# gooofy/zerovox

Measured on AMD Instinct MI355X. Metric: audio samples/sec + RTF, 128-phoneme zero-shot synth @22.05kHz, 1/2/4/8 GPU, higher is better.
Workload: dtype f16+bf16

## Files before the change

### zerovox_amd/csrc/gemm.hip

```cpp
#include "mfma_util.h"
#include "zvx_kernels.h"

#include <cstring>
#include <type_traits>

#ifndef ZVX_GEMM_PART
#define ZVX_GEMM_PART 0
#endif
#define ZVX_PART_MAIN (ZVX_GEMM_PART != 2)
#define ZVX_PART_RESFUSE (ZVX_GEMM_PART != 1)
#if ZVX_GEMM_PART == 2
extern thread_local bool zvx_gemm_dry_run;
#else
thread_local hipEvent_t zvx_gemm_ev_start = nullptr, zvx_gemm_ev_stop = nullptr;
thread_local bool zvx_gemm_dry_run = false;
#endif
#define g_dry_run zvx_gemm_dry_run

#define ZVX_LAUNCH(...) do { if (!g_dry_run) ZVX_DISPATCH(__VA_ARGS__); } while (0)

namespace zvx {


#define PITCH 80
// ... 478 lines not shown
    }
#pragma unroll
    for (int j = 0; j < TM; j++)
#pragma unroll
        for (int p = 0; p < NP; p++) {
            const int r = row_base + j * 32 + p * RPP + lane / LPR;
            if (r < a.M && r < out_len && nok) *(u32x4*)(obase + (long)r * a.ldo) = o[j][p];
        }
}

#if ZVX_PART_MAIN
#define SLAB_KC 64
#define SLAB_PITCH 144

__global__ void k_pack_w(const unsigned short* w, int ntaps, int N, int K, unsigned short* out, int nkc, long total_frag_lanes) {
    long idx = (long)blockIdx.x * blockDim.x + threadIdx.x;
    if (idx >= total_frag_lanes) return;
    const int lane = idx & 63; long t = idx >> 6;
    const int k16 = t & 3; t >>= 2;
    const int tap = t % ntaps; t /= ntaps;
    const int kc = t % nkc; const int nt = t / nkc;
    const int n = nt * 32 + (lane & 31);
    const int k0 = kc * SLAB_KC + k16 * 16 + 8 * (lane >> 5);
    unsigned short v[8];
#pragma unroll
    for (int e = 0; e < 8; e++) {
        const int k = k0 + e;
        v[e] = (n < N && k < K) ? w[((long)tap * N + n) * K + k] : (unsigned short)0;
    }
    uint4 o;
    o.x = v[0] | ((unsigned)v[1] << 16); o.y = v[2] | ((unsigned)v[3] << 16);
    o.z = v[4] | ((unsigned)v[5] << 16); o.w = v[6] | ((unsigned)v[7] << 16);
    *(uint4*)(out + idx * 8) = o;
}

size_t packed_weight_elems(int ntaps, int N, int K) {
    const int nkc = (K + SLAB_KC - 1) / SLAB_KC, nt = (N + 31) / 32;
    return (size_t)nt * nkc * ntaps * 4 * 64 * 8;
}
void launch_pack_weights(const void* w_bf16, int ntaps, int N, int K, void* out, hipStream_t s) {
    const int nkc = (K + SLAB_KC - 1) / SLAB_KC, nt = (N + 31) / 32;
    const long total = (long)nt * nkc * ntaps * 4 * 64;
    hipLaunchKernelGGL(k_pack_w, dim3((unsigned)((total + 255) / 256)), dim3(256), 0, s, (const unsigned short*)w_bf16, ntaps, N, K,
                       (unsigned short*)out, nkc, total);
}

void launch_pack_pair(const void* packedA, int ntapsA, int KA, const void* packedB, int ntapsB, int KB, int N, void* out, hipStream_t s) {
    const size_t nt = (N + 31) / 32;
    const size_t szA = (size_t)((KA + SLAB_KC - 1) / SLAB_KC) * ntapsA * 4 * 1024, szB = (size_t)((KB + SLAB_KC - 1) / SLAB_KC) * ntapsB * 4 * 1024;
    (void)hipMemcpy2DAsync(out, szA + szB, packedA, szA, szA, nt, hipMemcpyDeviceToDevice, s);
    (void)hipMemcpy2DAsync((char*)out + szA, szA + szB, packedB, szB, szB, nt, hipMemcpyDeviceToDevice, s);
}

template <int BM, int BN, int WM, int WN, bool FULLK, int MINW, int R, int EPI = -1, int MAXH = 64, bool F16 = false>
__global__ __launch_bounds__(256, MINW) void convslab_kernel(const GemmArgs a) {
    constexpr int TM = BM / WM / 32, TN = BN / WN / 32;
    constexpr int NIT = ((BM + MAXH) * 8 + 255) / 256;
    static_assert(WM * WN == 4, "4 waves");
    extern __shared__ __attribute__((aligned(16))) unsigned char slab[];
    if (F16 && EPI >= 0 && EPI != ZVX_EPI(0, 0, 1) && EPI != ZVX_EPI_FLIP) f16_saturate_mode();

    const int tid = threadIdx.x, lane = tid & 63, wave = __builtin_amdgcn_readfirstlane(tid >> 6);
    const int wr = wave % WM, wc = wave / WM;
    const int ntn = (a.N + BN - 1) / BN;
    int wg, b;
    if (a.xcd_flat) {
        const int nx = gridDim.x, nwg = nx * gridDim.y, id = blockIdx.y * nx + blockIdx.x, q = nwg >> 3, r = nwg & 7, xcd = id & 7;
        const int w = (xcd < r ? xcd * (q + 1) : r * (q + 1) + (xcd - r) * q) + (id >> 3);
        b = w / nx; wg = w - b * nx;
    } else {
        const int nwg = gridDim.x, id = blockIdx.x, q = nwg >> 3, r = nwg & 7, xcd = id & 7;
        wg = (xcd < r ? xcd * (q + 1) : r * (q + 1) + (xcd - r) * q) + (id >> 3);
        b = blockIdx.y;
    }
    const int nt = wg % ntn, mt = wg / ntn;
    const int m0 = mt * BM, n0 = nt * BN;
    const bool bflat = a.bflat != 0;
    const int out_len = bflat ? a.M : (a.out_len ? a.out_len[b] : a.M);
    const int in_len = bflat ? 0 : (a.in_len ? a.in_len[b] : a.in_len_static);
    if (m0 >= out_len || m0 >= a.M) return;
    if (bflat) {
        const int b0 = m0 / a.bflat, t0 = m0 - b0 * a.bflat;
        if (t0 >= a.out_len[b0] && t0 + BM <= a.bflat) return;
    }

    const int HL = a.halo_l, SR = BM + a.halo_l + a.halo_r;
    const int nkc = (a.K + SLAB_KC - 1) / SLAB_KC, n16 = a.K >> 4, ntaps = a.ntaps;
    const unsigned short* Xp = (const unsigned short*)a.X + (long)b * a.x_bs;
    const int nkc2 = (!FULLK && a.K2 > 0) ? (a.K2 + SLAB_KC - 1) / SLAB_KC : 0, n16_2 = a.K2 >> 4;
    const unsigned short* Xp2 = (const unsigned short*)a.X2 + (long)b * a.x2_bs;
    const int in_rows = ((MAXH > 64 || bflat) && a.flat_win) ? a.flat_rows : in_len;
    unsigned rowmask = 0xffffffffu;
    if (bflat) {
        rowmask = 0;
#pragma unroll
        for (int it = 0; it < NIT; it++) {
            const int g = m0 - HL + ((tid + it * 256) >> 3);
            if (g >= 0 && g < in_rows) { const int bb = g / a.bflat; if (g - bb * a.bflat < a.in_len[bb]) rowmask |= 1u << it; }
        }
    } else if (MAXH > 64 && a.flat_win) {
        rowmask = 0;
#pragma unroll
        for (int it = 0; it < NIT; it++) {
            const int g = m0 - HL + ((tid + it * 256) >> 3);
            if (g >= 0 && g < in_rows && (g % a.flat_win) < in_len) rowmask |= 1u << it;
        }
    }
// ... 2 lines not shown
#pragma unroll
    for (int i = 0; i < TN; i++)
#pragma unroll
        for (int j = 0; j < TM; j++)
#pragma unroll
            for (int e = 0; e < 16; e++) acc[i][j][e] = 0.f;

    constexpr bool WREG = R == 0;
    constexpr int F = BN / 32, CNT = F >= 4 ? F / 4 : 1, WD = 4, D = WREG ? WD : R - 1, WAITN = WREG ? (WD - 1) * TN : (D - 2) * CNT;
    const int nt32_total = (a.N + 31) >> 5;
    const int nsteps = a.ntaps * 4, gtotal = nkc * nsteps + nkc2 * 4;
    const uint4* wsrc[CNT];
#pragma unroll
    for (int j = 0; j < CNT; j++) {
        const int f = wave * CNT + j, t32 = (n0 >> 5) + f;
        wsrc[j] = (const uint4*)a.Wp + (long)(t32 < nt32_total ? t32 : 0) * gtotal * 64 + lane;
    }
    const int xrow0 = HL + wr * (BM / WM) + (lane & 31);
    const int koff = (lane >> 5) * 16;
    unsigned char* ring = slab + ((SR * SLAB_PITCH + 1023) & ~1023);
    const unsigned lds_base = (unsigned)(size_t)(__attribute__((address_space(3))) unsigned char*)slab;
    const int dvreg = a.dv[lane & (ZVX_MAX_TAPS - 1)];
    const bool loader = wave * CNT < F;
    const unsigned char* wq[TN];
#pragma unroll
    for (int i = 0; i < TN; i++) {
        const int t32 = (n0 >> 5) + wc * TN + i;
        wq[i] = (const unsigned char*)a.Wp + (long)(t32 < nt32_total ? t32 : 0) * gtotal * 1024;
    }
    const bool wave_dead = __builtin_amdgcn_readfirstlane((int)(n0 + wc * TN * 32 >= a.N)) != 0;
    const unsigned lane16 = lane * 16;
    u32x4 wreg[WREG ? WD : 1][TN] = {};
    auto wload = [&](int gs, int slot) {
        const long off = (long)(gs < gtotal ? gs : gtotal - 1) * 1024;
#pragma unroll
        for (int i = 0; i < TN; i++)
            asm volatile("global_load_dwordx4 %0, %1, %2" : "+v"(wreg[WREG ? slot : 0][i]) : "v"(lane16), "s"(wq[i] + off) : "memory");
    };
    auto dma = [&](int gs) {
        if (WREG || !loader) return;
        const int slot = gs & (R - 1);
        const long off = (long)(gs < gtotal ? gs : gtotal - 1) * 64;
#pragma unroll
        for (int j = 0; j < CNT; j++)
            __builtin_amdgcn_global_load_lds((const __attribute__((address_space(1))) void*)(wsrc[j] + off),
                                             (__attribute__((address_space(3))) void*)(ring + (slot * F + wave * CNT + j) * 1024), 16, 0, 0);
    };
    if (WREG) { wload(0, 0); wload(1, 1); wload(2, 2); wload(3, 3); }
    else {
#pragma unroll
        for (int s0 = 0; s0 < D; s0++) dma(s0);
    }

    for (int kc = 0; kc < nkc + nkc2; kc++) {
        const bool src2 = !FULLK && kc >= nkc;
        const unsigned short* const Xs = src2 ? Xp2 : Xp;
        const int ldxs = src2 ? a.ldx2 : a.ldx, Ks = src2 ? a.K2 : a.K, kbase = (src2 ? kc - nkc : kc) * SLAB_KC;
        {
            constexpr int FCH = NIT > 10 ? (NIT + 1) / 2 : NIT;
#pragma unroll
            for (int h0 = 0; h0 < NIT; h0 += FCH) {
                uint4 sv[FCH];
#pragma unroll
                for (int i = 0; i < FCH; i++) {
                    const int it = h0 + i;
                    const int c = tid + it * 256;
                    const int row = c >> 3, q = c & 7;
                    const int g = m0 - HL + row, k = kbase + q * 8;
                    sv[i] = make_uint4(0, 0, 0, 0);
                    if (it < NIT && c < SR * 8 && g >= 0 && g < in_rows && k < Ks && ((rowmask >> it) & 1)) sv[i] = *(const uint4*)(Xs + (long)g * ldxs + k);
                }
                if (kc && h0 == 0) __syncthreads();
#pragma unroll
                for (int i = 0; i < FCH; i++) {
                    const int c = tid + (h0 + i) * 256;
                    if (h0 + i < NIT && c < SR * 8) *(uint4*)(slab + (c >> 3) * SLAB_PITCH + (c & 7) * 16) = sv[i];
                }
            }
        }
        __syncthreads();
        int nk16 = 4;
        if (!FULLK) { nk16 = src2 ? n16_2 - (kc - nkc) * 4 : n16 - kc * 4; if (nk16 > 4) nk16 = 4; if (wave_dead) nk16 = 0; }
        const int ntaps_kc = src2 ? 1 : ntaps;

        uint4 xA[TM], wA[TN], xB[TM], wB[TN];
        const unsigned ring_rd = lds_base + (unsigned)(size_t)(ring - slab) + lane * 16 + wc * TN * 1024;
        const int gs0 = src2 ? nkc * nsteps + (kc - nkc) * 4 : kc * nsteps;
        auto rd = [&](uint4 (&xf)[TM], uint4 (&wf)[TN], int gs, unsigned rowoff, int kk) {
            if (!WREG) {
                const unsigned wa = ring_rd + (gs & ((WREG ? 1 : R) - 1)) * (F * 1024);
#pragma unroll
                for (int i = 0; i < TN; i++)
                    asm volatile("ds_read_b128 %0, %1 offset:%2" : "=v"(wf[i]) : "v"(wa), "n"(i * 1024));
            }
#pragma unroll
            for (int j = 0; j < TM; j++)
                asm volatile("ds_read_b128 %0, %1" : "=v"(xf[j]) : "v"(lds_base + rowoff + j * 32 * SLAB_PITCH + kk * 32));
        };
        auto mma = [&](uint4 (&xf)[TM], uint4 (&wf)[TN]) {
#pragma unroll
            for (int i = 0; i < TN; i++)
#pragma unroll
                for (int j = 0; j < TM; j++)
                    acc[i][j] = F16 ? __builtin_amdgcn_mfma_f32_32x32x16_f16(__builtin_bit_cast(f16x8, wf[i]), __builtin_bit_cast(f16x8, xf[j]), acc[i][j], 0, 0, 0)
                                    : __builtin_amdgcn_mfma_f32_32x32x16_bf16(__builtin_bit_cast(bf16x8, wf[i]),
                                                                       __builtin_bit_cast(bf16x8, xf[j]), acc[i][j], 0, 0, 0);
        };
        auto mma_r = [&](uint4 (&xf)[TM], int slot) {
#pragma unroll
            for (int i = 0; i < TN; i++)
#pragma unroll
                for (int j = 0; j < TM; j++)
                    acc[i][j] = F16 ? __builtin_amdgcn_mfma_f32_32x32x16_f16(__builtin_bit_cast(f16x8, wreg[WREG ? slot : 0][i]), __builtin_bit_cast(f16x8, xf[j]), acc[i][j], 0, 0, 0)
                                    : __builtin_amdgcn_mfma_f32_32x32x16_bf16(__builtin_bit_cast(bf16x8, wreg[WREG ? slot : 0][i]),
                                                                       __builtin_bit_cast(bf16x8, xf[j]), acc[i][j], 0, 0, 0);
        };
        auto rowoff_of = [&](int tap) {
            const int d = src2 ? 0 : __builtin_amdgcn_readlane(dvreg, tap < ntaps ? tap : ntaps - 1);
            return (unsigned)((xrow0 + d) * SLAB_PITCH + koff);
        };
        unsigned rowoff = rowoff_of(0);
        rd(xA, wA, gs0, rowoff, 0);
        for (int tap = 0; tap < ntaps_kc; tap++) {
            const unsigned rowoff_next = rowoff_of(tap + 1);
#pragma unroll
            for (int kk = 0; kk < 4; kk++) {
                const int gs = gs0 + tap * 4 + kk;
                if (WREG) asm volatile("s_waitcnt vmcnt(%0)" :: "n"(WAITN) : "memory");
                else asm volatile("s_waitcnt vmcnt(%0)\n\ts_barrier" :: "n"(WAITN) : "memory");
                dma(gs + D);
                if (kk & 1) rd(xA, wA, gs + 1, kk == 3 ? rowoff_next : rowoff, (kk + 1) & 3);
                else        rd(xB, wB, gs + 1, rowoff, kk + 1);
                asm volatile("s_waitcnt lgkmcnt(%0)" :: "n"(WREG ? TM : TM + TN) : "memory");
                __builtin_amdgcn_sched_barrier(0);
                if (FULLK || kk < nk16) {
                    if (WREG) { if (kk & 1) mma_r(xB, kk); else mma_r(xA, kk); }
                    else { if (kk & 1) mma(xB, wB); else mma(xA, wA); }
                }
                __builtin_amdgcn_sched_barrier(0);
                if (WREG) wload(gs + WD, kk);
            }
            rowoff = rowoff_next;
        }
        asm volatile("s_waitcnt lgkmcnt(0)" ::: "memory");
    }
    if (WREG) {
#pragma unroll
        for (int sl = 0; sl < (WREG ? WD : 1); sl++)
#pragma unroll
            for (int i = 0; i < TN; i++) asm volatile("s_waitcnt vmcnt(0)" : "+v"(wreg[sl][i]) :: "memory");
    } else {
        asm volatile("s_waitcnt vmcnt(0)" ::: "memory");
    }
    __syncthreads();
    if (EPI == ZVX_EPI_FLIP)
        epilogue_direct<TM, TN, !F16>(a, acc, b, m0 + wr * (BM / WM), n0 + wc * (BN / WN), out_len, lane, slab + wave * (32 * (TN * 64 + 16)));
    else if (EPI == ZVX_EPI(0, 0, 1))
        epilogue_direct<TM, TN, F16>(a, acc, b, m0 + wr * (BM / WM), n0 + wc * (BN / WN), out_len, lane, slab + wave * (32 * (TN * 64 + 16)));
    else
        epilogue_rows<TM, TN, 0, EPI, (F16 && EPI >= 0)>(a, acc, b, m0 + wr * (BM / WM), n0 + wc * (BN / WN), out_len, lane, slab + wave * (32 * (TN * 32 * 4 + 16)));
}

template <int C, int NT, int BM, int WM, int WN, int MINW, int MAXH = 64, bool F16 = false>
__global__ __launch_bounds__(256, MINW) void convreg_kernel(const GemmArgs a) {
    constexpr int TM = BM / WM / 32;
    constexpr int KS = C / 16;
    constexpr int PITCH_ = C * 2 + 16;
    constexpr int CPR = C / 8;
    constexpr int NIT = ((BM + MAXH) * CPR + 255) / 256;
    constexpr int FCH = NIT > 12 ? 8 : NIT;
    static_assert(WM * WN == 4 && WN * 32 == C, "wave layout");
    extern __shared__ __attribute__((aligned(16))) unsigned char slab[];

    const int tid = threadIdx.x, lane = tid & 63, wave = tid >> 6;
    const int wr = wave % WM, wc = wave / WM;
    int wg;
    {
        const int nwg = gridDim.x, id = blockIdx.x, q = nwg >> 3, r = nwg & 7, xcd = id & 7;
        wg = (xcd < r ? xcd * (q + 1) : r * (q + 1) + (xcd - r) * q) + (id >> 3);
    }
    const int m0 = wg * BM, b = blockIdx.y;
    const int out_len = a.out_len ? a.out_len[b] : a.M;
    const int in_len = a.in_len ? a.in_len[b] : a.in_len_static;
    if (m0 >= out_len || m0 >= a.M) return;
    const int HL = a.halo_l, SR = BM + a.halo_l + a.halo_r;
    const unsigned short* Xp = (const unsigned short*)a.X + (long)b * a.x_bs;

    uint4 w[NT][KS];
    {
        const uint4* Wq = (const uint4*)a.Wp + ((long)wc * NT * 4) * 64 + lane;
#pragma unroll
        for (int t = 0; t < NT; t++)
#pragma unroll
            for (int kk = 0; kk < KS; kk++) w[t][kk] = Wq[(t * 4 + kk) * 64];
    }
    {
        const bool flat = MAXH > 64 && a.flat_win;
// ... 882 lines not shown
    a.fused = 1;
    if (a.N == 128 && a.no_pairstream != 1) {
        const int h2 = (a.ntaps - 1) / 2, dil = a.dv1[1] - a.dv1[0];
        bool ok = a.alpha == 1.f && a.bias_mode == 1 && !a.post_scale && (!a.out || a.out_dtype == a.dtype) && a.res_mode == 2 && a.res_dtype == a.dtype &&
                  a.res == a.X && a.r_bs == a.x_bs && a.ldr == a.ldx && (!a.accum || a.accum_dtype == a.dtype) && (a.act == ACT_NONE || a.act == ACT_LRELU) &&
                  (a.accum_mode || a.out_scale == 1.f) && a.in_len == a.out_len;
        for (int t = 0; t < a.ntaps; t++) ok = ok && a.dv[t] == t - h2 && a.dv1[t] == (t - h2) * dil;
        if (ok) {
            PairArgs p;
            memset(&p, 0, sizeof p);
            p.X = a.X; p.x_bs = a.x_bs; p.ldx = a.ldx; p.W1 = a.Wp2; p.W2 = a.Wp; p.b1 = a.bias1; p.b2 = a.bias;
            p.C = a.N; p.ntaps = a.ntaps; p.dil = dil;
            p.out = a.out; p.o_bs = a.o_bs; p.ldo = a.ldo;
            p.accum = a.accum; p.a_bs = a.a_bs; p.lda = a.lda; p.accum_mode = a.accum ? a.accum_mode : 0;
            p.slope1 = a.slope1; p.res_inv_slope = a.res_inv_slope; p.out_scale = a.out_scale; p.slope = a.act == ACT_LRELU ? a.slope : 1.f;
            p.f16 = a.dtype == DT_F16;
            p.len = a.out_len; p.M = a.M; p.nbatch = a.nbatch; p.force = a.no_pairstream == 2;
            if (launch_pairstream(p, stream, g_dry_run)) return 23;
        }
    }
    {
        if (a.N == 32 && launch_resfuse_persist_c<32>(a, stream)) return 16;
        if (a.N == 64 && a.ntaps != 11 && launch_resfuse_persist_c<64>(a, stream)) return 17;
        if (a.N == 64 && a.ntaps == 11 && launch_resfuse_persist_c<64, 1>(a, stream)) return 17;
    }
    return -1;
}
#endif
#if ZVX_PART_MAIN

struct Variant { const char* name; int dt, bm, bn; };
static const Variant kVariants[] = {
    {"gemm_bf16_128x128", DT_BF16, 128, 128}, {"gemm_bf16_256x64", DT_BF16, 256, 64},
    {"gemm_bf16_256x32", DT_BF16, 256, 32},   {"gemm_f32_128x128", DT_F32, 128, 128},
    {"gemm_f32_256x64", DT_F32, 256, 64},     {"gemm_f32_256x32", DT_F32, 256, 32},
    {"convslab_bf16_128x256", DT_BF16, 128, 256}, {"convslab_bf16_256x128", DT_BF16, 256, 128},
    {"convslab_bf16_256x64", DT_BF16, 256, 64},   {"convslab_bf16_256x32", DT_BF16, 256, 32},
    {"(unused)", DT_BF16, 0, 0}, {"resfuse_bf16_c8", DT_BF16, 256, 8}, {"resfuse_bf16_c16", DT_BF16, 256, 16}, {"resfuse_bf16_c128", DT_BF16, 64, 128},
    {"convreg_bf16_c32", DT_BF16, 512, 32},       {"convreg_bf16_c64", DT_BF16, 256, 64},
    {"resfuse_bf16_c32", DT_BF16, 256, 32},       {"resfuse_bf16_c64", DT_BF16, 128, 64},
    {"gemm_bf16_64x64", DT_BF16, 64, 64},         {"gemm_f32_64x64", DT_F32, 64, 64},
    {"resstream_bf16_c32", DT_BF16, 64, 32},      {"resstream_bf16_c64", DT_BF16, 32, 64},
    {"convslab_bf16_128x128", DT_BF16, 128, 128},
    {"pairstream_bf16_c128", DT_BF16, 128, 128},
    {"narrowstage_c16", DT_BF16, 256, 16}, {"narrowstage_c8", DT_BF16, 512, 8},
    {"conv2d_persist_c32", DT_BF16, 384, 32}, {"conv2d_persist_c64", DT_BF16, 256, 64},
    {"conv2d_s2_c32", DT_BF16, 256, 64}, {"conv2d_s2_c64", DT_BF16, 128, 128},
    {"rb2fuse_bf16_c32", DT_BF16, 256, 32}, {"rb2fuse_bf16_c64", DT_BF16, 256, 64},
};
const char* gemm_variant_name(int id) { return kVariants[id].name; }
int gemm_num_variants() { return (int)(sizeof(kVariants) / sizeof(kVariants[0])); }


template <int BM, int BN, int WM, int WN, int MINW, int R, int EPI = -1>
static void launch_slab_variant(const GemmArgs& a, dim3 grid, size_t lds, hipStream_t stream) {
    const bool fullk = a.K % SLAB_KC == 0 && a.K2 == 0;
    if constexpr (R == 0 || EPI == -1 || EPI == ZVX_EPI(0, 0, 1) || EPI == ZVX_EPI_FLIP) {
        if (a.dtype == DT_F16) {
            if (fullk) ZVX_LAUNCH((convslab_kernel<BM, BN, WM, WN, true, MINW, R, EPI, 64, true>), grid, dim3(256), lds, stream, a);
            else if constexpr (EPI != ZVX_EPI_FLIP) ZVX_LAUNCH((convslab_kernel<BM, BN, WM, WN, false, MINW, R, EPI, 64, true>), grid, dim3(256), lds, stream, a);
            return;
        }
    }
    if constexpr (EPI < 0 || !(EPI & 16)) {
        if (fullk) ZVX_LAUNCH((convslab_kernel<BM, BN, WM, WN, true, MINW, R, EPI>), grid, dim3(256), lds, stream, a);
        else if constexpr (EPI != ZVX_EPI_FLIP) ZVX_LAUNCH((convslab_kernel<BM, BN, WM, WN, false, MINW, R, EPI>), grid, dim3(256), lds, stream, a);
    }
}

int gemm_epi_mode_of(const GemmArgs& a) {
    if (a.alpha == 1.f && !a.post_scale && a.out && a.out_dtype != a.dtype && a.dtype != DT_F32 && a.out_dtype != DT_F32 && !a.out_split3 && a.bias_mode == 1 && a.bias &&
        (a.act == ACT_NONE || a.act == ACT_LRELU) && !a.res_mode && !(a.accum && a.accum_mode) && a.out_scale == 1.f && a.K % SLAB_KC == 0 && !a.K2) return ZVX_EPI_FLIP;
    if (a.alpha != 1.f || a.post_scale || (a.out && a.out_dtype != a.dtype) || a.dtype == DT_F32 || a.out_split3 || a.bias_mode == 2) return -1;
    const int am = a.accum ? a.accum_mode : 0;
    if (a.dtype == DT_F16 && a.out && !am && a.act == ACT_NONE && a.res_mode <= 1 && (!a.res_mode || a.res_dtype == DT_F16) && (a.res_mode || a.out_scale != 1.f) &&
        (a.bias_mode == 0 || a.bias)) return ZVX_EPI_DEC(a.res_mode ? 1 : 0);
    if (a.bias_mode != 1 || !a.bias) return -1;
    if (a.act != ACT_NONE && a.act != ACT_LRELU) return -1;
    if (a.res_mode && (a.res_mode != 2 || a.res_dtype != a.dtype)) return -1;
    if (am && a.accum_dtype != a.dtype) return -1;
    if (!am && a.out_scale != 1.f) return -1;
    if (!a.out && !(am & 2)) return -1;
    const int e = ZVX_EPI(a.res_mode ? 1 : 0, am, a.out ? 1 : 0);
    switch (e) {
        case ZVX_EPI(0, 0, 1): case ZVX_EPI(1, 0, 1): case ZVX_EPI(1, 2, 0): case ZVX_EPI(1, 3, 0): case ZVX_EPI(1, 1, 1): return e;
    }
    return -1;
}

static int launch_convslab(GemmArgs a, hipStream_t stream) {
    const bool bflat_hint = a.bflat != 0;
    if (a.K2) {
        if (!a.X2 || a.K2 % 16 || a.ldx2 % 8 || a.flat_win || (a.bflat && a.x2_bs != (long)a.bflat * a.ldx2)) return -5;
    }
    if (a.bflat) {
        int h = 0;
        for (int i = 0; i < a.ntaps; i++) { const int d = a.dv[i] < 0 ? -a.dv[i] : a.dv[i]; if (d > h) h = d; }
        const bool ok = a.in_len && a.out_len && a.nbatch > 1 && a.bflat >= a.M + h && a.x_bs == (long)a.bflat * a.ldx && (!a.out || a.o_bs == (long)a.bflat * a.ldo) &&
                        (!a.res_mode || a.r_bs == (long)a.bflat * a.ldr) && !a.accum_mode && a.bias_mode != 2 && !a.flat_win && a.M > 128 && a.N >= 128 &&
                        (long)a.nbatch * a.bflat < (1l << 30);
        if (!ok) a.bflat = 0;
    }
    const int g_slab_small = a.slab_small & 7;
    int hl = 0, hr = 0;
    for (int i = 0; i < a.ntaps; i++) { hl = a.dv[i] < -hl ? -a.dv[i] : hl; hr = a.dv[i] > hr ? a.dv[i] : hr; }
    a.halo_l = hl; a.halo_r = hr;
    if (a.flat_win && !a.bflat) {
        if (a.N == a.K && (a.N == 32 || a.N == 64) && !(a.slab_small & 32) && a.dtype == DT_BF16 && a.ntaps == 9 && a.in_len && !a.out_len && hl == a.flat_win + 1 && hr == hl &&
            a.flat_win >= 64 && (long)a.flat_rows * a.ldx * 2 < 0x7fffffffL &&
// ... 229 lines not shown
```

### zerovox_amd/csrc/zvx.hip

```cpp
#include "../../include/zvx.h"
#include "zvx_kernels.h"

#include <dlfcn.h>
#include <math.h>
#include <cmath>
#include <rccl/rccl.h>
#include <stdarg.h>
#include <stdio.h>
#include <string.h>

#include <algorithm>
#include <map>
#include <sstream>
#include <stdexcept>
#include <string>
#include <vector>

using namespace zvx;

namespace {

struct ZvxError : std::runtime_error {
    int code;
    ZvxError(int c, const std::string& m) : std::runtime_error(m), code(c) {}
// ... 36 lines not shown
    hipStream_t front_stream = nullptr;
    hipEvent_t ev_front_done = nullptr, ev_mel_free = nullptr, ev_main_join = nullptr;
    int front_overlap = 1;
    bool mel_free_pending = false;
    bool front_dirty_main = true;
    struct HostSlot { void* p = nullptr; size_t cap = 0; hipEvent_t ready = nullptr, done = nullptr; bool pending = false; int B = 0, pcm16 = 0; long stride = 0, need = 0; };
    HostSlot host_slot[2];
    int host_next = 0, host_last = -1;
    hipStream_t copy_stream = nullptr;
    bool copy_is_comm = false;
    hipStream_t aux_stream = nullptr;
    hipEvent_t ev_aux[2] = {nullptr, nullptr};
    int va_overlap_maxb = 1 << 20;
    ncclComm_t comm = nullptr;
    int rank = 0, world = 1;
    hipEvent_t ev_compute = nullptr;
    std::map<const void*, hipEvent_t> gather_fence;
    std::string err;
    std::map<std::string, std::string> cfg;
    std::map<std::string, Tensor> tensors;
    std::vector<float> host_blob;
    std::map<std::string, DevBuf> bufs;
    std::map<const void*, const void*> packed;
    std::map<const void*, const void*> pair_packed;
    int dt = DT_BF16;
    int H = 0, emb_dim = 0, punct_dim = 0, n_phone_rows = 0, n_punct_rows = 0, max_txt_len = 0, max_mel_len = 0;
    int enc_layers = 0, enc_heads = 0, ffn_dim = 0, ffn_k0 = 0, ffn_k1 = 0, vp_dim = 0, vp_k = 0, n_bins = 0;
    int dec_layers = 0, dec_heads = 0, dec_scln = 0, n_mels = 0, hop = 0, res_dim = 0, dec_kind = 0, rn_asp = 1;
    std::vector<int> rn_layers, rn_filters, voc_rates, voc_ksizes, voc_rb_k;
    std::vector<std::vector<int>> voc_rb_d;
    int voc_resblock = 1, voc_c0 = 0;
    int B = 0, Tmax = 0, Lmax = 0;
    std::vector<int> T_host, mel_len_host;
    std::vector<int> in_stage;
    bool have_features = false, have_mel = false;
    int profile = 0;
    int profile_only = -1;
    int rs_prof = 0;
    int enc_split = 0;
    const void* fft_xs_ready = nullptr;
    int norm_fuse_maxb = 1 << 20;
    int dec_sc_fuse = 1;
    int dec_flat = 1;
    int voc_f16_stages = -1;
    int voc_h16_ok = -1;
    int voc_f16 = 1;
    int dec_f16 = 1;
    int use_attn_f32 = 1;
    int use_flash = 1;
    int use_resstream = 1;
    int rs_seg_min = 0;
    int spk_s2_fuse = 1;
    int spk_pool_fuse = 1;
    int slab_small = 2, slab_flat = 1;
    int poison_pads = 0;
    int sat_check = 0;
    unsigned long long* sat_count_dev() { return (unsigned long long*)buf("sat.count", 64); }
    void sat_scan(const void* x, int dt, long bs, int ld, int B, int rows_max, const int* rows, int C) {
        if (sat_check && x && dt == DT_F16) launch_count_sat16(x, bs, ld, B, rows_max, rows, C, sat_count_dev(), stream);
    }
    int use_rb2fuse = 1;
    int use_stagefuse = 1;
    struct NsWeights { void* W = nullptr; float* bias = nullptr; int woff[18] = {0}; };
    std::map<std::string, NsWeights> ns_weights;
    int use_pairstream = 1;
    int shape_log = 0;
    int max_frames = 1 << 18;
    int out_rate = 0;
    struct RsBank { int L = 0, M = 0, half = 0, T = 0, pitch = 0; const float* dev = nullptr; };
    std::map<std::pair<int, int>, RsBank> rs_banks;
    std::map<int, const double*> lim_wins;
    std::map<int, LoudCoef> loud_coefs;
    void* join_host = nullptr;
    size_t join_host_cap = 0;
    void* join_pinned(size_t bytes) {
        if (bytes > join_host_cap) {
            if (join_host) { HIPCHK(hipStreamSynchronize(stream)); HIPCHK(hipHostFree(join_host)); join_host = nullptr; join_host_cap = 0; }
            const size_t cap = bytes + bytes / 8 + 256;
            HIPCHK(hipHostMalloc(&join_host, cap, hipHostMallocDefault));
            join_host_cap = cap;
        }
        return join_host;
    }
    hipEvent_t stage_ev[ZVX_T_COUNT][2];
    bool stage_used[ZVX_T_COUNT];
    float stage_ms[ZVX_T_COUNT];
    std::vector<GemmEvent> pending;
    std::vector<zvx_kernel_stat> stats;
    std::string tag = "other";
    std::map<std::string, zvx_kernel_stat> tagstats;
    std::map<std::string, zvx_kernel_stat> namedstats;
    std::vector<hipEvent_t> event_pool;

    int cfg_int(const char* k) const {
        auto it = cfg.find(k);
        if (it == cfg.end()) fail(ZVX_E_MANIFEST, "manifest: missing cfg '%s'", k);
        return atoi(it->second.c_str());
    }
    std::vector<int> cfg_list(const char* k) const {
        auto it = cfg.find(k);
        if (it == cfg.end()) fail(ZVX_E_MANIFEST, "manifest: missing cfg '%s'", k);
        std::vector<int> v; std::stringstream ss(it->second); std::string tok;
        while (std::getline(ss, tok, ',')) if (!tok.empty()) v.push_back(atoi(tok.c_str()));
        return v;
    }
    const Tensor& t(const std::string& name) const {
// ... 46 lines not shown
    }
    void arena_end() {
        Arena& a = arena[arena_i];
        if (!a.cur || !stream) return;
        if (!a.ev) HIPCHK(hipEventCreateWithFlags(&a.ev, hipEventDisableTiming));
        HIPCHK(hipEventRecord(a.ev, stream));
        a.pending = true;
        arena_i ^= 1;
    }
    void upload(void* dst, const void* src, size_t bytes) {
        Arena& a = arena[arena_i];
        const size_t need = (bytes + 63) & ~(size_t)63;
        if (!a.p) { HIPCHK(hipHostMalloc((void**)&a.p, ARENA_BYTES, hipHostMallocDefault)); a.cap = ARENA_BYTES; }
        if (a.cur + need > a.cap) {
            HIPCHK(hipMemcpyAsync(dst, src, bytes, hipMemcpyHostToDevice, stream));
            HIPCHK(hipStreamSynchronize(stream));
            return;
        }
        memcpy(a.p + a.cur, src, bytes);
        HIPCHK(hipMemcpyAsync(dst, a.p + a.cur, bytes, hipMemcpyHostToDevice, stream));
        a.cur += need;
    }
    int* upload_ints(const std::string& name, const int* v, size_t n) {
        int* d = ibuf(name, n);
        upload(d, v, n * sizeof(int));
        return d;
    }
    size_t es() const { return dtype_size(dt); }

    hipEvent_t new_event() {
        hipEvent_t e;
        if (!event_pool.empty()) { e = event_pool.back(); event_pool.pop_back(); return e; }
        HIPCHK(hipEventCreate(&e));
        return e;
    }
    void stage_begin(int s) { if (profile) { HIPCHK(hipEventRecord(stage_ev[s][0], stream)); } }
    void stage_end(int s) { if (profile) { HIPCHK(hipEventRecord(stage_ev[s][1], stream)); stage_used[s] = true; } }

    template <typename V, typename L, typename D>
    void profiled(V&& vid, L&& launch, D&& describe) {
        const bool prof = profile >= 2 && (profile_only < 0 || vid() == profile_only);
        if (!prof) { launch(); return; }
        GemmEvent ev{};
        ev.a = new_event(); ev.b = new_event();
        struct Armed { Armed(hipEvent_t a, hipEvent_t b) { profile_events(a, b); } ~Armed() { profile_events(nullptr, nullptr); } };
        ev.variant = [&] { Armed armed(ev.a, ev.b); return launch(); }();
        describe(ev);
        ev.tag = tag;
        pending.push_back(ev);
    }
    void gemm(GemmArgs& a) {
        if (a.flops <= 0) a.flops = 2.0 * (double)a.M * a.nbatch * a.nheads * (double)a.N * ((double)a.K * a.ntaps + (double)a.K2);
        if (!a.Wp && a.dtype != DT_F32) { auto it = packed.find(a.W); if (it != packed.end()) a.Wp = it->second; }
        a.slab_small = slab_small | (spk_s2_fuse ? 0 : 32); a.xcd_flat = slab_flat;
        profiled([&] { return gemm_variant_of(a); }, [&] {
            const int id = a.fused == 2 ? launch_rb2fuse(a, stream) : (a.fused ? launch_resfuse(a, stream) : launch_gemm(a, stream));
            if (id < 0) fail(ZVX_E_INVALID, "launch_gemm rejected shape M=%d N=%d K=%d taps=%d", a.M, a.N, a.K, a.ntaps);
            return id;
        }, [&](GemmEvent& ev) {
            ev.flops = a.flops; ev.rows = (long)a.M * a.nbatch * a.nheads; ev.N = a.N; ev.K = a.K; ev.taps = a.ntaps; ev.res = a.res_mode; ev.fused = a.fused;
            const double esz = dtype_size(a.dtype);
            const double cells = (double)a.M * a.nbatch * a.nheads * a.N;
            ev.bytes = ((double)a.M * a.nbatch * a.nheads) * (double)(a.K + a.K2) * esz + (double)a.N * ((double)a.K * a.ntaps + a.K2) * esz * (a.fused ? 2 : 1) +
                       (a.out ? cells * dtype_size(a.out_dtype) : 0.0) + ((a.res_mode && !a.fused) ? cells * dtype_size(a.res_dtype) : 0.0) +
                       ((a.accum && (a.accum_mode & 1)) ? cells * dtype_size(a.accum_dtype) : 0.0) + ((a.accum && (a.accum_mode & 2)) ? cells * dtype_size(a.accum_dtype) : 0.0);
        });
        if (sat_check && a.nheads == 1) {
            sat_scan(a.out, a.out_dtype, a.o_bs, a.ldo, a.nbatch, a.M, a.out_len, a.N);
            if (a.accum && (a.accum_mode & 2)) sat_scan(a.accum, a.accum_dtype, a.a_bs, a.lda, a.nbatch, a.M, a.out_len, a.N);
        }
    }
    bool run_stream(StreamArgs& a) {
        const int id = launch_resstream(a, this->stream, true);
        if (id < 0) return false;
        profiled([&] { return id; }, [&] {
            const int id2 = launch_resstream(a, this->stream, false);
            if (id2 < 0) fail(ZVX_E_INVALID, "launch_resstream rejected a shape its dry run accepted (C=%d k=%d pairs=%d)", a.C, a.ntaps, a.npair);
            return id2;
        }, [&](GemmEvent& ev) {
            const double rows = (double)a.M * a.nbatch;
            ev.flops = 2.0 * 2.0 * a.npair * rows * a.C * a.C * a.ntaps; ev.rows = (long)rows; ev.N = a.C; ev.K = a.C; ev.taps = a.ntaps;
            ev.res = a.accum_mode; ev.fused = 10 + a.npair;
            ev.bytes = rows * a.C * 2.0 * (1 + (a.out ? 1 : 0) + ((a.accum && (a.accum_mode & 1)) ? 1 : 0) + ((a.accum && (a.accum_mode & 2)) ? 1 : 0));
        });
        return true;
    }
    template <typename F>
    void timed(double flops, double bytes, F&& f, const char* kname = nullptr) {
        const bool prof = profile >= 2 && profile_only < 0;
        GemmEvent ev{};
        if (prof) { ev.a = new_event(); ev.b = new_event(); HIPCHK(hipEventRecord(ev.a, stream)); }
        f();
        if (prof) { HIPCHK(hipEventRecord(ev.b, stream)); ev.variant = -1; ev.flops = flops; ev.bytes = bytes; ev.tag = tag; if (kname) ev.kname = kname; pending.push_back(ev); }
    }
    void resolve_events() {
        if (stats.empty()) {
            stats.resize(gemm_num_variants());
            for (int i = 0; i < gemm_num_variants(); i++) { memset(&stats[i], 0, sizeof stats[i]); snprintf(stats[i].name, 64, "%s", gemm_variant_name(i)); }
        }
        for (auto& e : pending) {
            float ms = 0.f;
            HIPCHK(hipEventElapsedTime(&ms, e.a, e.b));
            if (shape_log && e.variant >= 0) fprintf(stderr, "launch %-24s rows=%-8ld N=%-4d K=%-4d taps=%-2d res=%d fused=%d  %8.3f ms %8.1f TF/s %8.1f GB/s(alg)\n",
                                   gemm_variant_name(e.variant), e.rows, e.N, e.K, e.taps, e.res, e.fused, ms, e.flops / ms / 1e9, e.bytes / ms / 1e6);
            else if (shape_log) fprintf(stderr, "launch %-24s [%s]  %8.3f ms %8.1f GB/s(alg)\n", "(helper)", e.tag.c_str(), ms, e.bytes / ms / 1e6);
            if (e.variant >= 0) { auto& s = stats[e.variant]; s.launches++; s.ms += ms; s.flops += e.flops; s.bytes += e.bytes; }
            auto& ts = tagstats[e.tag];
// ... 2092 lines not shown
    for (auto& hs : c->host_slot) { if (hs.p) (void)hipHostFree(hs.p); if (hs.ready) (void)hipEventDestroy(hs.ready); if (hs.done) (void)hipEventDestroy(hs.done); }
    if (c->join_host) (void)hipHostFree(c->join_host);
    for (int i = 0; i < 2; i++) if (c->voc_aux[i]) { (void)hipStreamSynchronize(c->voc_aux[i]); (void)hipStreamDestroy(c->voc_aux[i]); }
    for (int i = 0; i < 3; i++) if (c->voc_ev[i]) (void)hipEventDestroy(c->voc_ev[i]);
    if (c->aux_stream) { (void)hipStreamSynchronize(c->aux_stream); (void)hipStreamDestroy(c->aux_stream); (void)hipEventDestroy(c->ev_aux[0]); (void)hipEventDestroy(c->ev_aux[1]); }
    if (c->front_stream) {
        (void)hipStreamSynchronize(c->front_stream); (void)hipStreamDestroy(c->front_stream);
        (void)hipEventDestroy(c->ev_front_done); (void)hipEventDestroy(c->ev_mel_free); (void)hipEventDestroy(c->ev_main_join);
    }
    for (auto& kv : c->bufs) if (kv.second.base) (void)hipFree(kv.second.base);
    for (auto e : c->event_pool) (void)hipEventDestroy(e);
    if (c->stream) {
        for (int s = 0; s < ZVX_T_COUNT; s++) { (void)hipEventDestroy(c->stage_ev[s][0]); (void)hipEventDestroy(c->stage_ev[s][1]); }
        (void)hipStreamDestroy(c->stream);
    }
    delete c;
}

const char* zvx_last_error(const zvx_ctx* c) { return c ? c->err.c_str() : g_create_error.c_str(); }

namespace {

struct Switch { const char* key; int zvx_ctx::*v; bool (*ok)(int64_t); };
bool flag(int64_t v) { return v == 0 || v == 1; }
bool count(int64_t v) { return v >= 0 && v <= INT32_MAX; }
const Switch kSwitches[] = {
    {"profile", &zvx_ctx::profile, [](int64_t v) { return v >= 0 && v <= 2; }},
    {"profile_only", &zvx_ctx::profile_only, [](int64_t v) { return v >= -1 && v < gemm_num_variants(); }},
    {"shape_log", &zvx_ctx::shape_log, flag},
    {"rs_prof", &zvx_ctx::rs_prof, flag},
    {"f16_sat_check", &zvx_ctx::sat_check, flag},
    {"poison_pads", &zvx_ctx::poison_pads, flag},
    {"max_frames", &zvx_ctx::max_frames, [](int64_t v) { return v >= 1 && v <= (1 << 24); }},
    {"enc_split", &zvx_ctx::enc_split, [](int64_t v) { return v >= 0 && v <= 2; }},
    {"attn_f32", &zvx_ctx::use_attn_f32, flag},
    {"flash", &zvx_ctx::use_flash, flag},
    {"front_overlap", &zvx_ctx::front_overlap, [](int64_t v) { return v >= 0 && v <= 2; }},
    {"va_overlap_maxb", &zvx_ctx::va_overlap_maxb, count},
    {"dec_f16", &zvx_ctx::dec_f16, flag},
    {"dec_flat", &zvx_ctx::dec_flat, flag},
    {"dec_sc_fuse", &zvx_ctx::dec_sc_fuse, flag},
    {"norm_fuse_maxb", &zvx_ctx::norm_fuse_maxb, count},
    {"voc_f16", &zvx_ctx::voc_f16, flag},
    {"voc_f16_stages", &zvx_ctx::voc_f16_stages, [](int64_t v) { return v >= -1 && v <= INT32_MAX; }},
    {"voc_overlap_maxb", &zvx_ctx::voc_overlap_maxb, count},
    {"voc_overlap_frames", &zvx_ctx::voc_overlap_frames, count},
    {"stagefuse", &zvx_ctx::use_stagefuse, flag},
    {"rb2fuse", &zvx_ctx::use_rb2fuse, flag},
    {"resstream", &zvx_ctx::use_resstream, flag},
    {"rs_seg_min", &zvx_ctx::rs_seg_min, [](int64_t v) { return v >= -1 && v <= INT32_MAX; }},
    {"pairstream", &zvx_ctx::use_pairstream, [](int64_t v) { return v == -1 || v == 0 || v == 1 || v == 3; }},
    {"slab_small", &zvx_ctx::slab_small, [](int64_t v) { return (v & ~32) >= 0 && (v & ~32) <= 2; }},
    {"slab_flat", &zvx_ctx::slab_flat, flag},
    {"spk_pool_fuse", &zvx_ctx::spk_pool_fuse, flag},
    {"spk_s2_fuse", &zvx_ctx::spk_s2_fuse, flag},
    {"out_rate", &zvx_ctx::out_rate, count},
};
const Switch* find_switch(const char* key) {
    for (const Switch& s : kSwitches) if (!strcmp(s.key, key)) return &s;
    return nullptr;
}

}

int64_t zvx_get_int(const zvx_ctx* c, const char* key) {
    if (!c || !key) return -1;
    if (const Switch* s = find_switch(key)) return c->*s->v;
    const std::string k(key);
    if (k == "precision") return c->dt == DT_F32 ? 1 : 0;
    if (k == "hidden") return c->H;
    if (k == "n_mels") return c->n_mels;
    if (k == "hop") return c->hop;
    if (k == "device") return c->device;
    if (k == "dec_kind") return c->dec_kind;
    if (k == "Lmax") return c->Lmax;
    if (k == "f16_sat_events") {
        zvx_ctx* m = const_cast<zvx_ctx*>(c);
        unsigned long long n = 0;
        if (hipSetDevice(m->device) != hipSuccess) return -1;
        try { unsigned long long* d = m->sat_count_dev(); m->sync(); if (hipMemcpy(&n, d, sizeof n, hipMemcpyDeviceToHost) != hipSuccess) return -1; } catch (...) { return -1; }
        return (int64_t)n;
    }
    if (k == "host_slot") return c->host_last;
    if (k.rfind("variant_id:", 0) == 0) { for (int i = 0; i < gemm_num_variants(); i++) if (k.substr(11) == gemm_variant_name(i)) return i; return -1; }
    auto it = c->cfg.find(k);
    if (it != c->cfg.end()) return atoll(it->second.c_str());
    return -1;
}

zvx_status zvx_set_int(zvx_ctx* c, const char* key, int64_t value) {
    return guarded(c, [&] {
        if (!key) fail(ZVX_E_INVALID, "key is NULL");
        const Switch* s = find_switch(key);
        if (!s) fail(ZVX_E_INVALID, "unknown option '%s'", key);
        if (!s->ok(value)) fail(ZVX_E_INVALID, "option '%s' does not take the value %lld", key, (long long)value);
        const std::string k(key);
        if (k == "out_rate" && value) {
            int L = 1, M = 1;
            rs_pair(model_rate(c), (int)value, &L, &M);
            if ((int)value != model_rate(c)) rs_bank(c, L, M);
        }
        if (k == "profile" || k == "profile_only" || k == "f16_sat_check" || k == "front_overlap") c->sync();
        c->*s->v = (int)value;
        if (k == "f16_sat_check") HIPCHK(hipMemsetAsync(c->sat_count_dev(), 0, 64, c->stream));
        if (k == "front_overlap") c->front_dirty_main = true;
        if (k == "enc_split") {
// ... 474 lines not shown
```

Measured before the change: 345.2 million.

## Double-buffer the activation slab in convslab kernel to overlap next-chunk loads with MFMA

Adds a PIPE variant of the conv-slab GEMM kernel that keeps two LDS slab buffers and prefetches the next K-chunk's activation rows into registers during the current chunk's tap loop, writing them to the alternate buffer between taps. This removes the serialized global-load-then-barrier stage at the start of every K chunk. Launch logic selects the variant for register-ring tiles with BN=128 when LDS fits and there are multiple chunks, behind a new default-on slab_pipe switch. It costs doubled LDS per block, which may lower occupancy, plus extra registers and finely tuned vmcnt waits that risk correctness.

```diff
diff --git a/zerovox_amd/csrc/gemm.hip b/zerovox_amd/csrc/gemm.hip
--- a/zerovox_amd/csrc/gemm.hip
+++ b/zerovox_amd/csrc/gemm.hip
@@ -554,7 +554,7 @@
     (void)hipMemcpy2DAsync((char*)out + szA, szA + szB, packedB, szB, szB, nt, hipMemcpyDeviceToDevice, s);
 }
 
-template <int BM, int BN, int WM, int WN, bool FULLK, int MINW, int R, int EPI = -1, int MAXH = 64, bool F16 = false>
+template <int BM, int BN, int WM, int WN, bool FULLK, int MINW, int R, int EPI = -1, int MAXH = 64, bool F16 = false, bool PIPE = false>
 __global__ __launch_bounds__(256, MINW) void convslab_kernel(const GemmArgs a) {
     constexpr int TM = BM / WM / 32, TN = BN / WN / 32;
     constexpr int NIT = ((BM + MAXH) * 8 + 255) / 256;
@@ -663,32 +663,85 @@
         for (int s0 = 0; s0 < D; s0++) dma(s0);
     }
 
-    for (int kc = 0; kc < nkc + nkc2; kc++) {
+    static_assert(!PIPE || (WREG && MAXH == 64), "PIPE: register-ring tiles with the 64-row halo budget");
+    constexpr int NR = PIPE && TM * TN >= 8 ? (NIT + 3) / 4 : 1, PR = (NIT + NR - 1) / NR, NTAIL = NR > 1 ? NIT - PR : 1;
+    const unsigned slab2 = PIPE ? (unsigned)((SR * SLAB_PITCH + 1023) & ~1023) : 0u;
+    const int nchunks = nkc + nkc2;
+    unsigned rowok = 0;
+    if (PIPE) {
+#pragma unroll
+        for (int it = 0; it < NIT; it++) {
+            const int c = tid + it * 256, g = m0 - HL + (c >> 3);
+            if (c < SR * 8 && g >= 0 && g < in_rows && ((rowmask >> it) & 1)) rowok |= 1u << it;
+        }
+    }
+    u32x4 sv[PIPE ? PR : 1] = {};
+    auto sreq = [&](auto& regs, int kc2, int it0) {
+        constexpr int N = PIPE ? (int)(sizeof(regs) / sizeof(regs[0])) : 0;
+        const bool s2 = !FULLK && kc2 >= nkc;
+        const unsigned short* const Xs = s2 ? Xp2 : Xp;
+        const unsigned ldxs = s2 ? a.ldx2 : a.ldx;
+        const int Ks = s2 ? a.K2 : a.K, k = (s2 ? kc2 - nkc : kc2) * SLAB_KC + (tid & 7) * 8;
+        const unsigned rows = k < Ks ? rowok >> it0 : 0u;
+#pragma unroll
+        for (int i = 0; i < N; i++) {
+            const unsigned g = (unsigned)(m0 - HL + ((tid + (it0 + i) * 256) >> 3));
+            const unsigned off = ((rows >> i) & 1) ? (g * ldxs + (unsigned)k) * 2u : 0u;
+            asm volatile("global_load_dwordx4 %0, %1, %2" : "+v"(regs[i]) : "v"(off), "s"(Xs) : "memory");
+        }
+    };
+    auto sput = [&](auto& regs, int kc2, int it0, unsigned dst) {
+        constexpr int N = PIPE ? (int)(sizeof(regs) / sizeof(regs[0])) : 0;
+        const bool s2 = !FULLK && kc2 >= nkc;
+        const unsigned rows = (s2 ? kc2 - nkc : kc2) * SLAB_KC + (tid & 7) * 8 < (s2 ? a.K2 : a.K) ? rowok >> it0 : 0u;
+        const unsigned wa = lds_base + dst + (unsigned)(((tid >> 3) + it0 * 32) * SLAB_PITCH + (tid & 7) * 16);
+#pragma unroll
+        for (int i = 0; i < N; i++) {
+            asm volatile("" : "+v"(regs[i]));
+            if (!((rows >> i) & 1)) regs[i] = (u32x4){0u, 0u, 0u, 0u};
+            if (tid + (it0 + i) * 256 < SR * 8) asm volatile("ds_write_b128 %0, %1 offset:%2" :: "v"(wa), "v"(regs[i]), "n"(i * 32 * SLAB_PITCH) : "memory");
+        }
+    };
+
+    auto stage = [&](int kc, const unsigned short* Xs, int ldxs, int Ks, int kbase) {
+        constexpr int FCH = NIT > 10 ? (NIT + 1) / 2 : NIT;
+#pragma unroll
+        for (int h0 = 0; h0 < NIT; h0 += FCH) {
+            uint4 sv[FCH];
+#pragma unroll
+            for (int i = 0; i < FCH; i++) {
+                const int it = h0 + i;
+                const int c = tid + it * 256;
+                const int row = c >> 3, q = c & 7;
+                const int g = m0 - HL + row, k = kbase + q * 8;
+                sv[i] = make_uint4(0, 0, 0, 0);
+                if (it < NIT && c < SR * 8 && g >= 0 && g < in_rows && k < Ks && ((rowmask >> it) & 1)) sv[i] = *(const uint4*)(Xs + (long)g * ldxs + k);
+            }
+            if (kc && h0 == 0) __syncthreads();
+#pragma unroll
+            for (int i = 0; i < FCH; i++) {
+                const int c = tid + (h0 + i) * 256;
+                if (h0 + i < NIT && c < SR * 8) *(uint4*)(slab + (c >> 3) * SLAB_PITCH + (c & 7) * 16) = sv[i];
+            }
+        }
+    };
+    if (PIPE) stage(0, Xp, a.ldx, a.K, 0);
+
+    for (int kc = 0; kc < nchunks; kc++) {
         const bool src2 = !FULLK && kc >= nkc;
         const unsigned short* const Xs = src2 ? Xp2 : Xp;
         const int ldxs = src2 ? a.ldx2 : a.ldx, Ks = src2 ? a.K2 : a.K, kbase = (src2 ? kc - nkc : kc) * SLAB_KC;
-        {
-            constexpr int FCH = NIT > 10 ? (NIT + 1) / 2 : NIT;
-#pragma unroll
-            for (int h0 = 0; h0 < NIT; h0 += FCH) {
-                uint4 sv[FCH];
-#pragma unroll
-                for (int i = 0; i < FCH; i++) {
-                    const int it = h0 + i;
-                    const int c = tid + it * 256;
-                    const int row = c >> 3, q = c & 7;
-                    const int g = m0 - HL + row, k = kbase + q * 8;
-                    sv[i] = make_uint4(0, 0, 0, 0);
-                    if (it < NIT && c < SR * 8 && g >= 0 && g < in_rows && k < Ks && ((rowmask >> it) & 1)) sv[i] = *(const uint4*)(Xs + (long)g * ldxs + k);
-                }
-                if (kc && h0 == 0) __syncthreads();
-#pragma unroll
-                for (int i = 0; i < FCH; i++) {
-                    const int c = tid + (h0 + i) * 256;
-                    if (h0 + i < NIT && c < SR * 8) *(uint4*)(slab + (c >> 3) * SLAB_PITCH + (c & 7) * 16) = sv[i];
-                }
-            }
-        }
+        const unsigned cur = PIPE ? (kc & 1) * slab2 : 0u;
+        const bool more = PIPE && kc + 1 < nchunks;
+#if ZVX_SLAB_CUT
+        if (!PIPE && kc == 0)
+#else
+        if (!PIPE)
+#endif
+            stage(kc, Xs, ldxs, Ks, kbase);
+#if ZVX_SLAB_CUT
+        if (PIPE || kc == 0)
+#endif
         __syncthreads();
         int nk16 = 4;
         if (!FULLK) { nk16 = src2 ? n16_2 - (kc - nkc) * 4 : n16 - kc * 4; if (nk16 > 4) nk16 = 4; if (wave_dead) nk16 = 0; }
@@ -728,7 +781,7 @@
         };
         auto rowoff_of = [&](int tap) {
             const int d = src2 ? 0 : __builtin_amdgcn_readlane(dvreg, tap < ntaps ? tap : ntaps - 1);
-            return (unsigned)((xrow0 + d) * SLAB_PITCH + koff);
+            return (unsigned)((xrow0 + d) * SLAB_PITCH + koff) + cur;
         };
         unsigned rowoff = rowoff_of(0);
         rd(xA, wA, gs0, rowoff, 0);
@@ -737,7 +790,10 @@
 #pragma unroll
             for (int kk = 0; kk < 4; kk++) {
                 const int gs = gs0 + tap * 4 + kk;
-                if (WREG) asm volatile("s_waitcnt vmcnt(%0)" :: "n"(WAITN) : "memory");
+                if (WREG) {
+                    if (kk && more && tap < NR) asm volatile("s_waitcnt vmcnt(%0)" :: "n"(WAITN + (PIPE ? PR : 0)) : "memory");
+                    else asm volatile("s_waitcnt vmcnt(%0)" :: "n"(WAITN) : "memory");
+                }
                 else asm volatile("s_waitcnt vmcnt(%0)\n\ts_barrier" :: "n"(WAITN) : "memory");
                 dma(gs + D);
                 if (kk & 1) rd(xA, wA, gs + 1, kk == 3 ? rowoff_next : rowoff, (kk + 1) & 3);
@@ -749,11 +805,29 @@
                     else { if (kk & 1) mma(xB, wB); else mma(xA, wA); }
                 }
                 __builtin_amdgcn_sched_barrier(0);
+                if (PIPE && kk == 0 && more) {
+                    if (tap && tap <= NR) sput(sv, kc + 1, (tap - 1) * PR, cur ^ slab2);
+                    if (tap < NR) sreq(sv, kc + 1, tap * PR);
+                }
                 if (WREG) wload(gs + WD, kk);
             }
             rowoff = rowoff_next;
         }
         asm volatile("s_waitcnt lgkmcnt(0)" ::: "memory");
+        if (more) {
+            if (ntaps_kc < NR) {
+                u32x4 tv[NTAIL] = {};
+                sreq(tv, kc + 1, ntaps_kc * PR);
+                asm volatile("s_waitcnt vmcnt(%0)" :: "n"(WD * TN + NTAIL) : "memory");
+                sput(sv, kc + 1, (ntaps_kc - 1) * PR, cur ^ slab2);
+                asm volatile("s_waitcnt vmcnt(0)" ::: "memory");
+                sput(tv, kc + 1, ntaps_kc * PR, cur ^ slab2);
+            } else if (ntaps_kc == NR) {
+                asm volatile("s_waitcnt vmcnt(%0)" :: "n"(WD * TN) : "memory");
+                sput(sv, kc + 1, (NR - 1) * PR, cur ^ slab2);
+            }
+            asm volatile("s_waitcnt lgkmcnt(0)" ::: "memory");
+        }
     }
     if (WREG) {
 #pragma unroll
@@ -1742,9 +1816,32 @@
 int gemm_num_variants() { return (int)(sizeof(kVariants) / sizeof(kVariants[0])); }
 
 
+#define ZVX_SLAB_PIPE_OFF 64
+#define ZVX_SLAB_PIPE_TAILK(BM, BN) ((BM) < 256)
 template <int BM, int BN, int WM, int WN, int MINW, int R, int EPI = -1>
 static void launch_slab_variant(const GemmArgs& a, dim3 grid, size_t lds, hipStream_t stream) {
     const bool fullk = a.K % SLAB_KC == 0 && a.K2 == 0;
+    if constexpr (R == 0 && BM >= 128 && BN == 128) {
+        const size_t one = ((size_t)(BM + a.halo_l + a.halo_r) * SLAB_PITCH + 1023) & ~(size_t)1023;
+        const int nchunks = (a.K + SLAB_KC - 1) / SLAB_KC + (a.K2 + SLAB_KC - 1) / SLAB_KC;
+        const long span = ((long)a.M + BM + 64) * (a.ldx > a.ldx2 ? a.ldx : a.ldx2) * 2;
+        if (!(a.slab_small & ZVX_SLAB_PIPE_OFF) && 4 * one <= (size_t)160 * 1024 && nchunks > 1 && span < (1l << 32) &&
+            (BM == 128 || a.ntaps >= 3)) {
+            const size_t lds2 = lds > 2 * one ? lds : 2 * one;
+            auto go = [&](auto kfn) {
+                if (lds2 > (size_t)64 * 1024 && !lds_opt_in((const void*)kfn)) return false;
+                ZVX_LAUNCH(kfn, grid, dim3(256), lds2, stream, a);
+                return true;
+            };
+            if (a.dtype == DT_F16) {
+                if (fullk) { if (go(convslab_kernel<BM, BN, WM, WN, true, MINW, R, EPI, 64, true, true>)) return; }
+                else if constexpr (EPI != ZVX_EPI_FLIP && ZVX_SLAB_PIPE_TAILK(BM, BN)) { if (go(convslab_kernel<BM, BN, WM, WN, false, MINW, R, EPI, 64, true, true>)) return; }
+            } else if constexpr (EPI < 0 || !(EPI & 16)) {
+                if (fullk) { if (go(convslab_kernel<BM, BN, WM, WN, true, MINW, R, EPI, 64, false, true>)) return; }
+                else if constexpr (EPI != ZVX_EPI_FLIP && ZVX_SLAB_PIPE_TAILK(BM, BN)) { if (go(convslab_kernel<BM, BN, WM, WN, false, MINW, R, EPI, 64, false, true>)) return; }
+            }
+        }
+    }
     if constexpr (R == 0 || EPI == -1 || EPI == ZVX_EPI(0, 0, 1) || EPI == ZVX_EPI_FLIP) {
         if (a.dtype == DT_F16) {
             if (fullk) ZVX_LAUNCH((convslab_kernel<BM, BN, WM, WN, true, MINW, R, EPI, 64, true>), grid, dim3(256), lds, stream, a);
diff --git a/zerovox_amd/csrc/zvx.hip b/zerovox_amd/csrc/zvx.hip
--- a/zerovox_amd/csrc/zvx.hip
+++ b/zerovox_amd/csrc/zvx.hip
@@ -112,6 +112,7 @@
     int rs_seg_min = 0;
     int spk_s2_fuse = 1;
     int spk_pool_fuse = 1;
+    int slab_pipe = 1;
     int slab_small = 2, slab_flat = 1;
     int poison_pads = 0;
     int sat_check = 0;
@@ -264,7 +265,7 @@
     void gemm(GemmArgs& a) {
         if (a.flops <= 0) a.flops = 2.0 * (double)a.M * a.nbatch * a.nheads * (double)a.N * ((double)a.K * a.ntaps + (double)a.K2);
         if (!a.Wp && a.dtype != DT_F32) { auto it = packed.find(a.W); if (it != packed.end()) a.Wp = it->second; }
-        a.slab_small = slab_small | (spk_s2_fuse ? 0 : 32); a.xcd_flat = slab_flat;
+        a.slab_small = slab_small | (spk_s2_fuse ? 0 : 32) | (slab_pipe ? 0 : 64); a.xcd_flat = slab_flat;
         profiled([&] { return gemm_variant_of(a); }, [&] {
             const int id = a.fused == 2 ? launch_rb2fuse(a, stream) : (a.fused ? launch_resfuse(a, stream) : launch_gemm(a, stream));
             if (id < 0) fail(ZVX_E_INVALID, "launch_gemm rejected shape M=%d N=%d K=%d taps=%d", a.M, a.N, a.K, a.ntaps);
@@ -2463,6 +2464,7 @@
     {"pairstream", &zvx_ctx::use_pairstream, [](int64_t v) { return v == -1 || v == 0 || v == 1 || v == 3; }},
     {"slab_small", &zvx_ctx::slab_small, [](int64_t v) { return (v & ~32) >= 0 && (v & ~32) <= 2; }},
     {"slab_flat", &zvx_ctx::slab_flat, flag},
+    {"slab_pipe", &zvx_ctx::slab_pipe, flag},
     {"spk_pool_fuse", &zvx_ctx::spk_pool_fuse, flag},
     {"spk_s2_fuse", &zvx_ctx::spk_s2_fuse, flag},
     {"out_rate", &zvx_ctx::out_rate, count},
```

New measurement: 341.6 million. -1.0%, worse.
